# joeyee/Onet

Hardware: AMD Instinct MI355X
Metric: training images/sec (twin 256x256 pass) (higher is better)
Workload: dtype f32

## Files before the change

include/onet_hip.h:

```cpp
#ifndef ONET_HIP_H
#define ONET_HIP_H

#include <stdint.h>

#ifdef __cplusplus
extern "C" {
#endif

#define ONET_OK 0
#define ONET_EINVAL (-1)
#define ONET_EHIP (-2)

const char* onet_last_error(void);
int onet_abi_version(void);
int onet_device_info(int* cu_count, int* lds_bytes, int* wave_size, char* arch, int arch_len);

int onet_conv3x3_pack_weights(const float* w, float* wp_fwd, float* wp_dgrad,
                              int Cout, int Cin, void* stream);
int onet_convT2x2_pack_weights(const float* w, float* wp_fwd, float* wp_dgrad,
                               int Cin, int Cout, void* stream);
int onet_convT2x2_pack_weights_fused(const float* w, float* wq, int Cin, int Cout, void* stream);
int onet_convT2x2_fwd(const float* x, int64_t x_bs, const float* wq, const float* bias, float* y, int64_t y_bs,
                      int B, int Cin, int Ct, int h, int w, int Ho, int Wo, int pt, int pl, int operand_bf16,
        void* stream);
// ... 3 lines not shown
int64_t onet_convT2x2_dgrad_dbias_ws_bytes(int B, int Ct, int h, int w);
int onet_convT2x2_dgrad_dbias(const float* dy, int64_t dy_bs, const float* wp_dgrad, float* dx, int64_t dx_bs, float* dbias,
                              void* ws, int64_t ws_bytes, int B, int Cin, int Ct, int h, int w, int Ho, int Wo, int pt, int pl, int operand_bf16,
        void* stream);
int64_t onet_convT2x2_wgrad_ws_bytes(int B, int Cin, int Ct, int h, int w);
int onet_convT2x2_wgrad(const float* x, int64_t x_bs, const float* dy, int64_t dy_bs, float* dw, void* ws,
                        int64_t ws_bytes, int B, int Cin, int Ct, int h, int w, int Ho, int Wo, int pt, int pl, int operand_bf16,
        void* stream);
int onet_convT2x2_dbias(const float* dy, int64_t dy_bs, float* dbias, double* scratch, int accumulate, int B,
                        int C, int h, int w, int Ho, int Wo, int pt, int pl, void* stream);

int onet_conv_fwd(const float* x, int64_t x_bs, const float* wp, float* z, int64_t z_bs,
                  float* bn_part, int B, int Cin, int Cout, int H, int W, int ks, void* stream);
int onet_conv_fwd_nparts(int B, int Cout, int H, int W);

int onet_conv3x3_pack_weights_winograd4(const float* w, float* wq_fwd, float* wq_dgrad,
                                        int Cout, int Cin, void* stream);
int onet_conv3x3_winograd4_fwd(const float* x, int64_t x_bs, const float* wq, float* z, int64_t z_bs,
                               int B, int Cin, int Cout, int H, int W, void* stream);
int onet_conv3x3_winograd4_nparts(int B, int H, int W);
int onet_conv3x3_winograd4_fwd_stats(const float* x, int64_t x_bs, const float* wq, float* z, int64_t z_bs,
                                     float* part, int B, int Cin, int Cout, int H, int W, void* stream);
int onet_conv3x3_winograd4_dgrad_bnreduce(const float* dz, int64_t dz_bs, const float* wq_dgrad, float* da,
                                          int64_t da_bs, const float* z_prev, int64_t z_prev_bs,
                                          const float* save_prev, int group_images, float* part2,
                                          int B, int Cdz, int Cda, int H, int W, void* stream);
int onet_convT2x2_fwd_p(const float* x, int64_t x_bs, const float* wq, const float* bias, void* yP, int64_t yP_bs, const void* y_amax,
                        int nparts, int B, int Cin, int Ct, int h, int w, int Ho, int Wo, int pt, int pl, int operand_bf16, void* stream);
int onet_convT2x2_pack_weights_slots(const float* w, void* wP, void* wdP, void* amax_ws, int Cin, int Ct, int nparts, void* stream);
int onet_convT2x2_fwd_slots(const void* xP, int64_t xP_bs, const void* x_amax, const void* wP, const float* bias, void* yP, int64_t yP_bs,
                            const void* y_amax, int nparts, int B, int Cin, int Ct, int h, int w, void* stream);
int onet_convT2x2_dgrad_slots(const void* dyP, int64_t dyP_bs, const void* dy_amax, const void* wdP, float* dx, int64_t dx_bs, int nparts, int B,
                              int Cin, int Ct, int h, int w, void* stream);
int64_t onet_convT2x2_wgrad_slots_ws_bytes(int B, int Cin, int Ct, int h, int w);
int onet_convT2x2_wgrad_slots(const void* xP, int64_t xP_bs, const void* x_amax, const void* dyP, int64_t dyP_bs, const void* dy_amax, float* dw,
                              float* dbias, void* ws, int64_t ws_bytes, int nparts, int B, int Cin, int Ct, int h, int w, void* stream);
int onet_convT2x2_out_bound(const float* w, const float* bias, int Cin, int Ct, const void* x_amax, void* y_amax, void* stream);

int onet_conv3x3_split_pack_weights(const float* w, void* wq_fwd, void* wq_dgrad, void* amax_ws, int Cout, int Cin, int fwd_f16,
                                    int dgrad_f16, void* stream);
int onet_absmax_slots(const float* x, int64_t n, void* slots, void* stream);
int onet_conv3x3_split_conv_amax(const float* x, int64_t x_bs, const void* x_amax, int scale_always, const void* wq, float* z, int64_t z_bs,
                                 float* part, int B, int Cin, int Cout, int H, int W, void* stream);
int onet_conv3x3_split_wgrad_f16(const float* x, int64_t x_bs, const void* x_amax, const float* save, int n_groups, const float* dz,
                                 int64_t dz_bs, const void* dz_amax, float* dw, void* ws, int64_t ws_bytes, int B, int Cin, int Cout,
                                 int H, int W, int accumulate, void* stream);
int onet_conv3x3_split_fwd(const float* x, int64_t x_bs, const void* wq, int wq_f16, float* z, int64_t z_bs, int B, int Cin, int Cout,
                           int H, int W, void* stream);
int onet_conv3x3_split_nparts(int B, int H, int W);
int onet_split_pack_act(const float* x, int64_t x_bs, void* xs, int64_t xs_bs, int B, int C, int H, int W, int f16, float scale,
                        const void* slots ,
                        void* stream);
int onet_conv3x3_split_dgrad_pre_bnreduce(const void* dzs, int64_t dzs_bs, const void* dz_amax, int scale_always, const void* wq, int wq_f16,
                                          float* da, int64_t da_bs, const void* z_prev, int z_bf16, int64_t z_bs, const float* save, int group_images,
                                          float* rec4, void* da_amax, int B, int Cin, int Cout, int H, int W, void* stream);
int onet_conv3x3_split_fwd_pre(const void* xs, int64_t xs_bs, const void* x_amax, int scale_always, const void* x_amax2, int split_ch,
                               const void* wq, int wq_f16, void* z, int z_bf16 , int64_t z_bs,
                               float* part, int B, int Cin, int Cout, int H, int W,
                               void* stream);
int onet_conv3x3_split_dgrad_pre_slots(const void* dzs, int64_t dzs_bs, const void* dz_amax, int scale_always, const void* wq, int wq_f16,
                                       float* da, int64_t da_bs, void* daP, int64_t daP_bs, int ch0, const void* daP_amax, int B, int Cin,
                                       int Cout, int H, int W, void* stream);
int onet_conv3x3_dgrad_bound(const float* w, int Cout, int Cin, int ci0, const void* dz_amax, void* out_slots, void* stream);
int onet_conv3x3_split_fwd_pre_act(const void* xs, int64_t xs_bs, const void* x_amax, int scale_always, const void* x_amax2, int split_ch,
                                   const void* wq, const float* save, void* aP, int64_t aP_bs, const void* aP_slots, void* a_amax, float* a,
                                   int64_t a_bs, int B, int Cin, int Cout, int H, int W, void* stream);
// ... 145 lines not shown
```

onet_amd/csrc/convt_gemm.hip:

```cpp
#include <algorithm>
#include <cstdlib>
#include "common.hpp"

using namespace onet;

typedef float f32x16 __attribute__((ext_vector_type(16)));
typedef float f32x4g __attribute__((ext_vector_type(4)));
typedef float f32x2g __attribute__((ext_vector_type(2)));
typedef int i32x4g __attribute__((ext_vector_type(4)));
typedef __bf16 bf16x8g __attribute__((ext_vector_type(8)));
typedef __bf16 bf16x2g __attribute__((ext_vector_type(2)));
typedef unsigned u32x4g __attribute__((ext_vector_type(4)));

namespace {

__device__ __forceinline__ i32x4g g_rsrc(const void* base, int64_t bytes) {
    const uint64_t p = reinterpret_cast<uint64_t>(base);
    i32x4g r;
    r.x = (int)(p & 0xffffffffu);
    r.y = (int)((p >> 32) & 0xffffu);
    r.z = bytes > 0x7fffffffll ? 0x7fffffff : (int)bytes;
    r.w = 0x00020000;
    return r;
}
__device__ __forceinline__ unsigned g_lds(const float* p) {
    return (unsigned)(uintptr_t)(__attribute__((address_space(3))) const float*)p;
}
__device__ __forceinline__ void g_dma16(i32x4g rsrc, unsigned lds_base, unsigned voff) {
    unsigned keep;
    asm volatile("s_nop 4\n\ts_mov_b32 %0, m0\n\ts_mov_b32 m0, %3\n\ts_nop 0\n\tbuffer_load_dwordx4 %1, %2, 0 offen lds\n\ts_mov_b32 m0, %0"
                 : "=&s"(keep)
                 : "v"(voff), "s"(rsrc), "s"(lds_base)
                 : "memory");
// ... 424 lines not shown

__global__ __launch_bounds__(256) void convt_dbias_reduce_kernel(const float* __restrict__ part, float* __restrict__ db, int ntiles, int Ct) {
    const int c = blockIdx.x;
    double s = 0.0;
    for (int t = threadIdx.x; t < ntiles; t += 256) s += (double)part[(int64_t)t * Ct + c];
    __shared__ double sh[4];
    double v[1] = {s};
    block_sum_256<double, 1>(v, sh);
    if (threadIdx.x == 0) db[c] = (float)v[0];
}


typedef _Float16 f16x8g __attribute__((ext_vector_type(8)));

struct SArgs {
    const void* wP;
    const void* xP;
    int64_t x_bs;
    const float* bias;
    void* yP;
    int64_t y_bs;
    const unsigned* x_slots;
    const unsigned* y_slots;
    int B, Cin, Ct, h, w, mTiles, nTiles;
};

template <int NP>
__device__ __forceinline__ f32x16 s_mfma(u32x4g a, u32x4g b, f32x16 c) {
    if constexpr (NP == 2) return __builtin_amdgcn_mfma_f32_32x32x16_f16(__builtin_bit_cast(f16x8g, a), __builtin_bit_cast(f16x8g, b), c, 0, 0, 0);
    else return __builtin_amdgcn_mfma_f32_32x32x16_bf16(__builtin_bit_cast(bf16x8g, a), __builtin_bit_cast(bf16x8g, b), c, 0, 0, 0);
}

constexpr int SLOT_NST = 2, SLOT_OCC = 4;
template <int N>
__device__ __forceinline__ void slot_wait() {
    asm volatile("s_waitcnt vmcnt(%0)" ::"n"(N) : "memory");
}

template <int NP>
__global__ __launch_bounds__(256, SLOT_OCC) void convt_slot_fwd_kernel(SArgs g) {
    constexpr int KS = 4 / NP;
    constexpr int TILE = KS * NP * 128;
    constexpr int NPC = TILE / 256;
    constexpr int NST = SLOT_NST;
    __shared__ __attribute__((aligned(16))) u32x4g lds[NST * 2 * TILE];
    const int bid = xcd_block_id();
    const int mt = bid % g.mTiles;
    const int nt = bid / g.mTiles;
    const int tid = threadIdx.x, lane = tid & 63, wid = __builtin_amdgcn_readfirstlane(tid >> 6);
    const int wr = wid >> 1, wc = wid & 1, l31 = lane & 31, kh = lane >> 5;
    const int hw = g.h * g.w, M = 4 * g.Ct;
    const int m0 = mt * 128, n0 = nt * 128;
    const int b = n0 / hw, p0 = n0 % hw;

    const i32x4g ra = g_rsrc(g.wP, (int64_t)(g.Cin / 8) * NP * M * 16);
    const i32x4g rb = g_rsrc(reinterpret_cast<const unsigned*>(g.xP) + (int64_t)b * g.x_bs, (int64_t)(g.Cin / 8) * hw * NP * 16);
    unsigned a_off[NPC], b_off[NPC];
#pragma unroll
    for (int j = 0; j < NPC; ++j) {
        const int s = (wid * NPC + j) * 64 + lane;
        const int c8 = s / (NP * 128), part = (s >> 7) % NP, r = s & 127;
        a_off[j] = (unsigned)((((int64_t)c8 * NP + part) * M + m0 + r) * 16);
        const int p = p0 + r, i = p / g.w, jx = p % g.w;
        b_off[j] = (unsigned)(((((int64_t)c8 * g.h + i) * NP + part) * g.w + jx) * 16);
    }
    const unsigned a_step = (unsigned)((int64_t)KS * NP * M * 16), b_step = (unsigned)((int64_t)KS * hw * NP * 16);
    const unsigned lds0 = (unsigned)(uintptr_t)(__attribute__((address_space(3))) u32x4g*)lds;
    auto issue = [&](int chunk, int buf) __attribute__((always_inline)) {
        const unsigned la = lds0 + (unsigned)(buf * 2 * TILE * 16), lb = la + TILE * 16;
#pragma unroll
        for (int j = 0; j < NPC; ++j) g_dma16(ra, la + (wid * NPC + j) * 1024, a_off[j] + chunk * a_step);
#pragma unroll
        for (int j = 0; j < NPC; ++j) g_dma16(rb, lb + (wid * NPC + j) * 1024, b_off[j] + chunk * b_step);
    };
    static_assert(NST >= 2 && NST <= 4, "the tail waits below cover rings of two to four stages");

    f32x16 acc[2][2];
#pragma unroll
    for (int t = 0; t < 2; ++t)
#pragma unroll
        for (int u = 0; u < 2; ++u)
#pragma unroll
            for (int r = 0; r < 16; ++r) acc[t][u][r] = 0.f;

    const int nch = g.Cin / (8 * KS);
#pragma unroll
    for (int c = 0; c < NST - 1; ++c) issue(c, c);
    float undo = 1.f;
    if constexpr (NP == 2) {
        const float* meta = reinterpret_cast<const float*>(reinterpret_cast<const _Float16*>(g.wP) + (int64_t)NP * g.Cin * M);
        float x_inv;
        (void)amax_scale(amax_read(g.x_slots), false, x_inv);
        undo = meta[1] * x_inv;
    }
    float s_inv;
    const float s_up = NP == 1 ? 1.f : amax_scale(amax_read(g.y_slots), false, s_inv);
    float bsv[2][4];
#pragma unroll
    for (int t = 0; t < 2; ++t)
#pragma unroll
        for (int gq = 0; gq < 4; ++gq) bsv[t][gq] = g.bias ? g.bias[(m0 + wr * 64 + t * 32 + 8 * gq + 4 * kh) >> 2] : 0.f;
    slot_wait<(NST - 2) * 2 * NPC>();
    __syncthreads();
    for (int c = 0; c < nch; ++c) {
        const int buf = c % NST;
        if (c + NST - 1 < nch) issue(c + NST - 1, (c + NST - 1) % NST);
        const u32x4g* A = lds + buf * 2 * TILE + wr * 64 + l31;
        const u32x4g* Bt = lds + buf * 2 * TILE + TILE + wc * 64 + l31;
#pragma unroll
        for (int s = 0; s < KS / 2; ++s) {
            u32x4g af[2][NP], bf[2][NP];
#pragma unroll
            for (int t = 0; t < 2; ++t)
#pragma unroll
                for (int q = 0; q < NP; ++q) af[t][q] = A[((2 * s + kh) * NP + q) * 128 + t * 32];
#pragma unroll
            for (int u = 0; u < 2; ++u)
#pragma unroll
                for (int q = 0; q < NP; ++q) bf[u][q] = Bt[((2 * s + kh) * NP + q) * 128 + u * 32];
            if constexpr (NP == 2) {
#pragma unroll
                for (int t = 0; t < 2; ++t)
#pragma unroll
                    for (int u = 0; u < 2; ++u) acc[t][u] = s_mfma<NP>(af[t][1], bf[u][0], acc[t][u]);
#pragma unroll
                for (int t = 0; t < 2; ++t)
#pragma unroll
                    for (int u = 0; u < 2; ++u) acc[t][u] = s_mfma<NP>(af[t][0], bf[u][1], acc[t][u]);
            }
#pragma unroll
            for (int t = 0; t < 2; ++t)
#pragma unroll
                for (int u = 0; u < 2; ++u) acc[t][u] = s_mfma<NP>(af[t][0], bf[u][0], acc[t][u]);
        }
        const int behind = min(NST - 2, nch - 2 - c);
        constexpr int PPC = 2 * NPC;
        if (behind >= 2) slot_wait<2 * PPC>();
        else if (behind == 1) slot_wait<1 * PPC>();
        else slot_wait<0>();
        __syncthreads();
    }

#pragma unroll
    for (int t = 0; t < 2; ++t)
#pragma unroll
        for (int u = 0; u < 2; ++u) {
            const int p = p0 + wc * 64 + u * 32 + l31, y = p / g.w, x = p % g.w;
            const int c8 = (m0 + wr * 64 + t * 32) >> 5;
            float px[2][8];
#pragma unroll
            for (int gq = 0; gq < 4; ++gq) {
                const float bs = bsv[t][gq];
#pragma unroll
                for (int dj = 0; dj < 2; ++dj) {
                    const unsigned d0 = __builtin_bit_cast(unsigned, fmaf(acc[t][u][4 * gq + dj], undo, bs));
                    const unsigned d1 = __builtin_bit_cast(unsigned, fmaf(acc[t][u][4 * gq + 2 + dj], undo, bs));
                    const auto sw = __builtin_amdgcn_permlane32_swap(d0, d1, false, false);
                    const unsigned even = sw[0], odd = sw[1];
                    px[dj][2 * gq] = __builtin_bit_cast(float, even);
                    px[dj][2 * gq + 1] = __builtin_bit_cast(float, odd);
                }
            }
            u32x4g* dst = reinterpret_cast<u32x4g*>(reinterpret_cast<unsigned*>(g.yP) + (int64_t)b * g.y_bs) +
                          ((int64_t)(c8 * (2 * g.h) + 2 * y + kh) * NP) * (2 * g.w) + 2 * x;
#pragma unroll
            for (int dj = 0; dj < 2; ++dj) {
                u32x4g hi, mid;
#pragma unroll
                for (int k = 0; k < 4; ++k) {
                    if constexpr (NP == 2) {
                        unsigned hh, mm;
                        split2h_s(px[dj][2 * k], px[dj][2 * k + 1], s_up, hh, mm);
                        hi[k] = hh;
                        mid[k] = mm;
                    } else {
                        hi[k] = g_pack(px[dj][2 * k], px[dj][2 * k + 1]);
                    }
                }
                dst[dj] = hi;
                if constexpr (NP == 2) dst[2 * g.w + dj] = mid;
            }
        }
}

struct SDArgs {
    const void* wdP;
    const void* dyP;
    int64_t dy_bs;
    float* dx;
    int64_t dx_bs;
    const unsigned* dy_slots;
    int B, Cin, Ct, h, w, mTiles, nTiles;
};

template <int NP>
__global__ __launch_bounds__(256, SLOT_OCC) void convt_slot_dgrad_kernel(SDArgs g) {
    constexpr int KS = 4 / NP;
    constexpr int TILE = KS * NP * 128;
    constexpr int NPC = TILE / 256;
    constexpr int NST = SLOT_NST;
    __shared__ __attribute__((aligned(16))) u32x4g lds[NST * 2 * TILE];
    const int bid = xcd_block_id();
    const int mt = bid % g.mTiles, nt = bid / g.mTiles;
    const int tid = threadIdx.x, lane = tid & 63, wid = __builtin_amdgcn_readfirstlane(tid >> 6);
    const int wr = wid >> 1, wc = wid & 1, l31 = lane & 31, kh = lane >> 5;
    const int hw = g.h * g.w, M = g.Cin, Ho = 2 * g.h, Wo = 2 * g.w;
    const int m0 = mt * 128, n0 = nt * 128;
    const int b = n0 / hw, p0 = n0 % hw;

    const i32x4g ra = g_rsrc(g.wdP, (int64_t)(g.Ct / 2) * NP * M * 16);
    const i32x4g rb = g_rsrc(reinterpret_cast<const unsigned*>(g.dyP) + (int64_t)b * g.dy_bs, (int64_t)(g.Ct / 8) * Ho * NP * Wo * 16);
    unsigned a_off[NPC], b_px[NPC];
    int b_ks[NPC];
#pragma unroll
    for (int j = 0; j < NPC; ++j) {
        const int s = (wid * NPC + j) * 64 + lane;
        const int ks = s / (NP * 128), part = (s >> 7) % NP, r = s & 127;
        a_off[j] = (unsigned)((((int64_t)ks * NP + part) * M + m0 + r) * 16);
        const int p = p0 + r, i = p / g.w, jx = p % g.w;
        b_px[j] = (unsigned)(((((int64_t)2 * i) * NP + part) * Wo + 2 * jx) * 16);
        b_ks[j] = ks;
    }
    const unsigned a_step = (unsigned)((int64_t)KS * NP * M * 16);
    const unsigned lds0 = (unsigned)(uintptr_t)(__attribute__((address_space(3))) u32x4g*)lds;
    auto issue = [&](int chunk, int buf) __attribute__((always_inline)) {
        const unsigned la = lds0 + (unsigned)(buf * 2 * TILE * 16), lb = la + TILE * 16;
#pragma unroll
        for (int j = 0; j < NPC; ++j) g_dma16(ra, la + (wid * NPC + j) * 1024, a_off[j] + chunk * a_step);
#pragma unroll
        for (int j = 0; j < NPC; ++j) {
            const int kq = chunk * KS + b_ks[j], c8 = kq >> 2, di = (kq >> 1) & 1, dj = kq & 1;
            g_dma16(rb, lb + (wid * NPC + j) * 1024, b_px[j] + (unsigned)((((int64_t)c8 * Ho + di) * NP * Wo + dj) * 16));
        }
    };

    f32x16 acc[2][2];
#pragma unroll
    for (int t = 0; t < 2; ++t)
#pragma unroll
        for (int u = 0; u < 2; ++u)
#pragma unroll
            for (int r = 0; r < 16; ++r) acc[t][u][r] = 0.f;

    const int nch = (g.Ct / 2) / KS;
#pragma unroll
    for (int c = 0; c < NST - 1; ++c) issue(c, c);
    float undo = 1.f;
    if constexpr (NP == 2) {
        const float* meta = reinterpret_cast<const float*>(reinterpret_cast<const _Float16*>(g.wdP) + (int64_t)NP * 4 * g.Ct * M);
        float dy_inv;
        (void)amax_scale(amax_read(g.dy_slots), true, dy_inv);
        undo = meta[1] * dy_inv;
    }
    slot_wait<(NST - 2) * 2 * NPC>();
    __syncthreads();
    for (int c = 0; c < nch; ++c) {
        const int buf = c % NST;
        if (c + NST - 1 < nch) issue(c + NST - 1, (c + NST - 1) % NST);
        const u32x4g* A = lds + buf * 2 * TILE + wr * 64 + l31;
        const u32x4g* Bt = lds + buf * 2 * TILE + TILE + wc * 64 + l31;
#pragma unroll
        for (int s = 0; s < KS / 2; ++s) {
            u32x4g af[2][NP], bf[2][NP];
#pragma unroll
            for (int t = 0; t < 2; ++t)
#pragma unroll
                for (int q = 0; q < NP; ++q) af[t][q] = A[((2 * s + kh) * NP + q) * 128 + t * 32];
#pragma unroll
            for (int u = 0; u < 2; ++u)
#pragma unroll
                for (int q = 0; q < NP; ++q) bf[u][q] = Bt[((2 * s + kh) * NP + q) * 128 + u * 32];
            if constexpr (NP == 2) {
#pragma unroll
                for (int t = 0; t < 2; ++t)
#pragma unroll
                    for (int u = 0; u < 2; ++u) acc[t][u] = s_mfma<NP>(af[t][1], bf[u][0], acc[t][u]);
#pragma unroll
                for (int t = 0; t < 2; ++t)
#pragma unroll
                    for (int u = 0; u < 2; ++u) acc[t][u] = s_mfma<NP>(af[t][0], bf[u][1], acc[t][u]);
            }
#pragma unroll
            for (int t = 0; t < 2; ++t)
#pragma unroll
                for (int u = 0; u < 2; ++u) acc[t][u] = s_mfma<NP>(af[t][0], bf[u][0], acc[t][u]);
        }
        const int behind = min(NST - 2, nch - 2 - c);
        constexpr int PPC = 2 * NPC;
        if (behind >= 2) slot_wait<2 * PPC>();
        else if (behind == 1) slot_wait<1 * PPC>();
        else slot_wait<0>();
        __syncthreads();
    }
    float* xb = g.dx + (int64_t)b * g.dx_bs;
#pragma unroll
    for (int t = 0; t < 2; ++t)
#pragma unroll
        for (int u = 0; u < 2; ++u) {
            const int p = p0 + wc * 64 + u * 32 + l31;
#pragma unroll
            for (int r = 0; r < 16; ++r) {
                const int ci = m0 + wr * 64 + t * 32 + (r & 3) + 8 * (r >> 2) + 4 * kh;
                xb[(int64_t)ci * hw + p] = acc[t][u][r] * undo;
            }
        }
}

struct SWArgs {
    const void* xP;
    int64_t x_bs;
    const void* dyP;
    int64_t dy_bs;
    float* slab;
    float* db_part;
    const unsigned* x_slots;
    const unsigned* dy_slots;
    int B, Cin, Ct, h, w, lw;
    int mTiles, nTiles, splitK, chunksPerSplit;
};

constexpr int SW_CP = 32;
// ... 382 lines not shown
    if (rc) return rc;
    hipLaunchKernelGGL(convt_wgrad_reduce_kernel, dim3((unsigned)cdiv(n / 4, 256)), dim3(256), 0, st, (const float*)ws, dw, g.splitK,
                       n / 4, 0);
    return check_launch("convt_wgrad_reduce_kernel");
}

}

static bool wgrad_slots_plan(int B, int Cin, int Ct, int h, int w, int& splitK, int& per) {
    const bool big = (Cin % 256) == 0 && (Ct % 64) == 0;
    const int64_t chunks = (int64_t)B * h * w / SW_CP;
    const int64_t tiles = big ? (int64_t)(Cin / 256) * (Ct / 64) : (int64_t)(Cin / 128) * (Ct / 32);
    int64_t k = std::max<int64_t>(1, ((big ? 256 : 512) + tiles - 1) / tiles);
    k = std::min<int64_t>(k, std::max<int64_t>(1, chunks / (512 / SW_CP)));
    k = std::min<int64_t>(k, std::max<int64_t>(1, (256ll << 20) / ((int64_t)Cin * 4 * Ct * 4)));
    per = (int)((chunks + k - 1) / k);
    splitK = (int)((chunks + per - 1) / per);
    return big;
}

template <int NP, int BIG>
static int launch_wgrad_slots(SWArgs g, hipStream_t st) {
    using C = SwCfg<BIG>;
    const int lds = NP * (C::APL + C::BPL) * C::PXP * 16 * C::NST;
    auto kern = convt_slot_wgrad_kernel<NP, BIG>;
    static PerDeviceOnce once;
    if (once.first()) (void)hipFuncSetAttribute(reinterpret_cast<const void*>(kern), hipFuncAttributeMaxDynamicSharedMemorySize, lds);
    const int64_t blocks = (int64_t)g.splitK * g.mTiles * g.nTiles;
    ONET_REQUIRE(blocks > 0 && blocks < (1ll << 31), "convT2x2_wgrad_slots: grid too large");
    hipLaunchKernelGGL(kern, dim3((unsigned)blocks), dim3(C::NWAVE * 64), lds, st, g);
    return check_launch("convt_slot_wgrad_kernel");
}

extern "C" {

int onet_convT2x2_pack_weights_slots(const float* w, void* wP, void* wdP, void* amax_ws, int Cin, int Ct, int nparts, void* stream) {
    ONET_REQUIRE(w && wP && Cin > 0 && Ct > 0 && (Cin % 8) == 0 && (!wdP || (Ct % 8) == 0) && (nparts == 1 || nparts == 2),
                 "convT2x2_pack_weights_slots: bad args");
    ONET_REQUIRE(nparts == 1 || amax_ws, "convT2x2_pack_weights_slots: the fp16 pack needs the 8 KB magnitude workspace");
    hipStream_t st = as_stream(stream);
    const int64_t n = (int64_t)Cin * 4 * Ct;
    if (nparts == 2) {
        (void)hipMemsetAsync(amax_ws, 0, AMAX_SLOTS * AMAX_STRIDE * sizeof(unsigned), st);
        hipLaunchKernelGGL(convt_absmax_kernel, dim3((unsigned)std::min<int64_t>((n + 1023) / 1024, 1024)), dim3(256), 0, st, w, n, (unsigned*)amax_ws);
        int rc = check_launch("convt_absmax_kernel");
        if (rc) return rc;
    }
    hipLaunchKernelGGL(convt_pack_slots_kernel, dim3((unsigned)std::min<int64_t>(((wdP ? 2 : 1) * n + 255) / 256, 8192)), dim3(256), 0, st, w, wP,
                       wdP, Cin, Ct, nparts, (const unsigned*)amax_ws);
    return check_launch("convt_pack_slots_kernel");
}

int onet_convT2x2_dgrad_slots(const void* dyP, int64_t dyP_bs, const void* dy_amax, const void* wdP, float* dx, int64_t dx_bs, int nparts, int B,
                              int Cin, int Ct, int h, int w, void* stream) {
    ONET_REQUIRE(dyP && wdP && dx && B > 0 && Cin > 0 && Ct > 0 && h > 0 && w > 0 && (nparts == 1 || nparts == 2), "convT2x2_dgrad_slots: bad args");
    const int64_t hw = (int64_t)h * w;
    if ((Cin % 128) || (Ct % 32) || (hw % 128) || (w & 1) || !aligned16(dyP) || !aligned16(wdP) || (dyP_bs & 3) ||
        (int64_t)Ct * 4 * hw * 2 * nparts >= (1ll << 31) || (int64_t)Cin * 4 * Ct * 2 * nparts >= (1ll << 31))
        return 1;
    ONET_REQUIRE(dyP_bs >= (int64_t)Ct * 4 * hw * nparts / 2 && dx_bs >= (int64_t)Cin * hw, "convT2x2_dgrad_slots: batch stride too small");
    SDArgs g{wdP, dyP, dyP_bs, dx, dx_bs, (const unsigned*)dy_amax, B, Cin, Ct, h, w, Cin / 128, (int)(B * hw / 128)};
    const int64_t blocks = (int64_t)g.mTiles * g.nTiles;
    ONET_REQUIRE(blocks > 0 && blocks < (1ll << 31), "convT2x2_dgrad_slots: grid too large");
    if (nparts == 2) hipLaunchKernelGGL(convt_slot_dgrad_kernel<2>, dim3((unsigned)blocks), dim3(256), 0, as_stream(stream), g);
    else hipLaunchKernelGGL(convt_slot_dgrad_kernel<1>, dim3((unsigned)blocks), dim3(256), 0, as_stream(stream), g);
    return check_launch("convt_slot_dgrad_kernel");
}

int64_t onet_convT2x2_wgrad_slots_ws_bytes(int B, int Cin, int Ct, int h, int w) {
    if ((Cin % 128) || (Ct % 32) || (((int64_t)h * w) % 128) || (w & (w - 1))) return 0;
    int k, per;
    (void)wgrad_slots_plan(B, Cin, Ct, h, w, k, per);
    return (int64_t)k * ((int64_t)Cin * 4 * Ct + 4 * Ct) * 4;
}

int onet_convT2x2_wgrad_slots(const void* xP, int64_t xP_bs, const void* x_amax, const void* dyP, int64_t dyP_bs, const void* dy_amax, float* dw,
                              float* dbias, void* ws, int64_t ws_bytes, int nparts, int B, int Cin, int Ct, int h, int w, void* stream) {
    ONET_REQUIRE(xP && dyP && dw && ws && B > 0 && Cin > 0 && Ct > 0 && h > 0 && w > 0 && (nparts == 1 || nparts == 2), "convT2x2_wgrad_slots: bad args");
    const int64_t hw = (int64_t)h * w;
    if ((Cin % 128) || (Ct % 32) || (hw % 128) || (w & (w - 1)) || w < 2 || !aligned16(xP) || !aligned16(dyP) || !aligned16(dw) || (xP_bs & 3) ||
        (dyP_bs & 3) || (int64_t)Cin * hw * 2 * nparts >= (1ll << 31) || (int64_t)Ct * 4 * hw * 2 * nparts >= (1ll << 31))
        return 1;
    ONET_REQUIRE(xP_bs >= (int64_t)Cin * hw * nparts / 2 && dyP_bs >= (int64_t)Ct * 4 * hw * nparts / 2, "convT2x2_wgrad_slots: batch stride too small");
    int lw = 0;
    while ((1 << lw) < w) ++lw;
    SWArgs g{xP, xP_bs, dyP, dyP_bs, (float*)ws, nullptr, (const unsigned*)x_amax, (const unsigned*)dy_amax, B, Cin, Ct, h, w, lw, 0, 0, 1, 0};
    const bool big = wgrad_slots_plan(B, Cin, Ct, h, w, g.splitK, g.chunksPerSplit);
    g.mTiles = big ? Cin / 256 : Cin / 128;
    g.nTiles = big ? Ct / 64 : Ct / 32;
    const int64_t n = (int64_t)Cin * 4 * Ct;
    ONET_REQUIRE(ws_bytes >= (int64_t)g.splitK * (n + 4 * Ct) * 4, "convT2x2_wgrad_slots: workspace too small (onet_convT2x2_wgrad_slots_ws_bytes)");
    if (dbias) g.db_part = (float*)ws + (int64_t)g.splitK * n;
    hipStream_t st = as_stream(stream);
    int rc;
    if (nparts == 2) rc = big ? launch_wgrad_slots<2, 1>(g, st) : launch_wgrad_slots<2, 0>(g, st);
    else rc = big ? launch_wgrad_slots<1, 1>(g, st) : launch_wgrad_slots<1, 0>(g, st);
    if (rc) return rc;
    hipLaunchKernelGGL(convt_wgrad_reduce_kernel, dim3((unsigned)cdiv(n / 4, 256)), dim3(256), 0, st, (const float*)ws, dw, g.splitK, n / 4, 0);
    rc = check_launch("convt_wgrad_reduce_kernel");
    if (rc || !dbias) return rc;
    hipLaunchKernelGGL(convt_dbias_reduce_kernel, dim3((unsigned)Ct), dim3(256), 0, st, (const float*)g.db_part, dbias, g.splitK * 4, Ct);
    return check_launch("convt_dbias_reduce_kernel");
}

int onet_convT2x2_fwd_slots(const void* xP, int64_t xP_bs, const void* x_amax, const void* wP, const float* bias, void* yP, int64_t yP_bs,
                            const void* y_amax, int nparts, int B, int Cin, int Ct, int h, int w, void* stream) {
    ONET_REQUIRE(xP && wP && yP && B > 0 && Cin > 0 && Ct > 0 && h > 0 && w > 0 && (nparts == 1 || nparts == 2), "convT2x2_fwd_slots: bad args");
    const int64_t hw = (int64_t)h * w;
    if ((Cin % 32) || Cin < 128 || (Ct % 32) || (hw % 128) || (w & 1) || !aligned16(xP) || !aligned16(wP) || !aligned16(yP) || (xP_bs & 3) || (yP_bs & 3) ||
        (int64_t)Cin * hw * 2 * nparts >= (1ll << 31) || (int64_t)Cin * 4 * Ct * 2 * nparts >= (1ll << 31))
        return 1;
    ONET_REQUIRE(xP_bs >= (int64_t)Cin * hw * nparts / 2 && yP_bs >= (int64_t)Ct * 4 * hw * nparts / 2, "convT2x2_fwd_slots: batch stride too small");
    SArgs g{wP, xP, xP_bs, bias, yP, yP_bs, (const unsigned*)x_amax, (const unsigned*)y_amax, B, Cin, Ct, h, w, (4 * Ct) / 128, (int)(B * hw / 128)};
    const int64_t blocks = (int64_t)g.mTiles * g.nTiles;
    ONET_REQUIRE(blocks > 0 && blocks < (1ll << 31), "convT2x2_fwd_slots: grid too large");
    if (nparts == 2) hipLaunchKernelGGL(convt_slot_fwd_kernel<2>, dim3((unsigned)blocks), dim3(256), 0, as_stream(stream), g);
    else hipLaunchKernelGGL(convt_slot_fwd_kernel<1>, dim3((unsigned)blocks), dim3(256), 0, as_stream(stream), g);
    return check_launch("convt_slot_fwd_kernel");
}

}
```

onet_amd/ops.py:

```python
from __future__ import annotations

import torch

from . import _lib

F32 = torch.float32


import os as _os


def _flags_from_env():
    out = {}
    for item in _os.environ.get("ONET_FLAGS", "").split(","):
        if "=" in item:
            k, v = item.split("=", 1)
            out[k.strip()] = v.strip()
    return out


_FLAGS = _flags_from_env()


def _flag(name, default):
# ... 307 lines not shown

def convT2x2_fwd(x, wq, bias, out, Ct, pt, pl):
    require_gpu(x, wq, out)
    x, xbs = plane(x)
    B, Cin, h, w = x.shape
    Ho, Wo = out.shape[2], out.shape[3]
    obs = out.stride(0) if B > 1 else Ct * Ho * Wo
    e0 = _prof_begin("convt_gemm_kernel")
    _lib.call("onet_convT2x2_fwd", _p(x), xbs, _p(wq), _p(bias), _p(out), obs, B, Cin, Ct, h, w, Ho, Wo, pt, pl,
              convt_operand_bf16(B, h, w, Ct), _stream())
    _prof_end("convt_gemm_kernel", 2.0 * B * h * w * Cin * 4 * Ct, e0, 4.0 * (B * h * w * (Cin + 4 * Ct) + 4 * Cin * Ct))


def convT2x2_out_bound(weight, bias, x_amax):
    w = weight.detach()
    w = w if w.is_contiguous() else w.contiguous()
    slots = new_amax(w.device)
    _lib.call("onet_convT2x2_out_bound", _p(w), _p(bias), w.shape[0], w.shape[1], _p(x_amax), _p(slots), _stream())
    return slots


def packT2x2_slots(w, parts=2, dgrad=False):
    require_gpu(w)
    w = w.detach().contiguous()
    Cin, Ct = w.shape[0], w.shape[1]
    dt = torch.float16 if parts == 2 else BF
    wP = torch.empty(Cin * 4 * Ct * parts + 4, dtype=dt, device=w.device)
    wdP = torch.empty(Cin * 4 * Ct * parts + 4, dtype=dt, device=w.device) if dgrad else None
    ws = torch.empty(2048, dtype=torch.int32, device=w.device) if parts == 2 else None
    _lib.call("onet_convT2x2_pack_weights_slots", _p(w), _p(wP), _p(wdP), _p(ws), Cin, Ct, parts, _stream())
    return (wP, wdP) if dgrad else wP


def convT2x2_dgrad_slots(dyP, wdP, Cin, dy_slots=None):
    B, C8, Ho, parts, Wo, _ = dyP.shape
    Ct, h, w = C8 * 8, Ho // 2, Wo // 2
    dx = torch.empty((B, Cin, h, w), dtype=F32, device=dyP.device)
    e0 = _prof_begin("convt_gemm_kernel")
    rc = _lib.load().onet_convT2x2_dgrad_slots(_p(dyP), _pbs(dyP), _p(dy_slots), _p(wdP), _p(dx), Cin * h * w, parts, B, Cin, Ct, h, w, _stream())
    flops, nb = 2.0 * B * h * w * Cin * 4 * Ct, B * h * w * (4.0 * Cin + 2.0 * parts * 4 * Ct)
    _prof_end("convt_gemm_kernel", flops if rc == 0 else 0.0, e0, nb if rc == 0 else 0.0)
    if rc < 0:
        raise _lib.OnetHipError(f"onet_convT2x2_dgrad_slots failed ({rc}): {_lib.last_error()}")
    return dx if rc == 0 else None


def convT2x2_wgrad_slots(xP, dyP, dw_shape, x_slots=None, dy_slots=None, want_dbias=False, out=None, db_out=None):
    B, C8, h, parts, w, _ = xP.shape
    Cin, Ct = C8 * 8, dyP.shape[1] * 8
    assert tuple(dw_shape) == (Cin, Ct, 2, 2) and dyP.shape[3] == parts and dyP.shape[2] == 2 * h and xP.dtype == dyP.dtype
    need = int(_lib.load().onet_convT2x2_wgrad_slots_ws_bytes(B, Cin, Ct, h, w))
    if need <= 0:
        return None
    ws = workspace(need, xP.device)
    dw = out if out is not None else torch.empty(dw_shape, dtype=F32, device=xP.device)
    db = (db_out if db_out is not None else torch.empty(Ct, dtype=F32, device=xP.device)) if want_dbias else None
    e0 = _prof_begin("convt_wgrad_gemm_kernel")
    rc = _lib.load().onet_convT2x2_wgrad_slots(_p(xP), _pbs(xP), _p(x_slots), _p(dyP), _pbs(dyP), _p(dy_slots), _p(dw), _p(db), _p(ws),
                                               ws.numel() * 4, parts, B, Cin, Ct, h, w, _stream())
    flops, nb = 2.0 * B * h * w * Cin * 4 * Ct, 2.0 * parts * B * h * w * (Cin + 4 * Ct)
    _prof_end("convt_wgrad_gemm_kernel", flops if rc == 0 else 0.0, e0, nb if rc == 0 else 0.0)
    if rc < 0:
        raise _lib.OnetHipError(f"onet_convT2x2_wgrad_slots failed ({rc}): {_lib.last_error()}")
    return (dw, db) if rc == 0 else None


def conv3x3_dgrad_bound(weight, dz_slots, ci0):
    w = weight.detach()
    w = w if w.is_contiguous() else w.contiguous()
    slots = new_amax(w.device)
# ... 59 lines not shown
                               f"{self._v} instead")

    def __getitem__(self, i):
        if self._t[i] is None:
            self._same_weight()
            self._t[i] = packT2x2_fused(self.w) if i == 0 else packT2x2(self.w)[1]
        return self._t[i]

    def __iter__(self):
        return iter((_LazyPack(self, 0), _LazyPack(self, 1)))

    def __len__(self):
        return 2

    def slots(self, parts):
        if parts not in self._s:
            self._same_weight()
            self._s[parts] = packT2x2_slots(self.w, parts, dgrad=bool(CONVT_BWD_SLOTS))
        v = self._s[parts]
        return v[0] if isinstance(v, tuple) else v

    def dgrad_slots(self, parts):
        v = self._s.get(parts)
        if not isinstance(v, tuple):
            self._same_weight()
            self._s[parts] = v = packT2x2_slots(self.w, parts, dgrad=True)
        return v[1]


def convT2x2_fwd_slots(xP, wP, bias, outP, Ct, x_slots=None, slots=None, kind="convt_gemm_kernel"):
    B, C8, h, parts, w, _ = xP.shape
    assert outP.shape[3] == parts and outP.shape[2] == 2 * h and outP.shape[4] == 2 * w and xP.dtype == wP.dtype == outP.dtype
    Cin = C8 * 8
    e0 = _prof_begin(kind)
    rc = _lib.load().onet_convT2x2_fwd_slots(_p(xP), _pbs(xP), _p(x_slots), _p(wP), _p(bias), _p(outP), _pbs(outP), _p(slots), parts, B, Cin, Ct,
                                             h, w, _stream())
    eb = 2.0 * parts
    flops, nb = 2.0 * B * h * w * Cin * 4 * Ct, eb * (B * h * w * (Cin + 4 * Ct) + 4 * Cin * Ct)
    _prof_end(kind, flops if rc == 0 else 0.0, e0, nb if rc == 0 else 0.0)
    if rc < 0:
        raise _lib.OnetHipError(f"onet_convT2x2_fwd_slots failed ({rc}): {_lib.last_error()}")
    return rc == 0


def convT2x2_fwd_p(x, wq, bias, outP, Ct, pt, pl, slots=None):
    require_gpu(x, wq)
    x, xbs = plane(x)
    B, Cin, h, w = x.shape
    Ho, Wo = outP.shape[2], outP.shape[4]
    e0 = _prof_begin("convt_gemm_kernel")
    rc = _lib.load().onet_convT2x2_fwd_p(_p(x), xbs, _p(wq), _p(bias), _p(outP), _pbs(outP), _p(slots), outP.shape[3], B, Cin, Ct, h, w, Ho, Wo, pt, pl,
                                         convt_operand_bf16(B, h, w, Ct), _stream())
    flops, nb = 2.0 * B * h * w * Cin * 4 * Ct, 4.0 * (B * h * w * (Cin + 4 * Ct) + 4 * Cin * Ct)
    _prof_end("convt_gemm_kernel", flops if rc == 0 else 0.0, e0, nb if rc == 0 else 0.0)
    if rc < 0:
        raise _lib.OnetHipError(f"onet_convT2x2_fwd_p failed ({rc}): {_lib.last_error()}")
    return rc == 0


import os as _os
CONV_ALGO = _os.environ.get("ONET_CONV_ALGO", "auto")
TWIN = _flag("TWIN", True)


BF = torch.bfloat16

# ... 1322 lines not shown
```

Measured before the change: 602.2.

## Add wide 256x128 tile variant for convT slot fwd/dgrad kernels with LDS-staged stores

```diff
diff --git a/include/onet_hip.h b/include/onet_hip.h
--- a/include/onet_hip.h
+++ b/include/onet_hip.h
@@ -59,6 +59,7 @@
                             const void* y_amax, int nparts, int B, int Cin, int Ct, int h, int w, void* stream);
 int onet_convT2x2_dgrad_slots(const void* dyP, int64_t dyP_bs, const void* dy_amax, const void* wdP, float* dx, int64_t dx_bs, int nparts, int B,
                               int Cin, int Ct, int h, int w, void* stream);
+int onet_convT2x2_slots_wide_tile(int enable);
 int64_t onet_convT2x2_wgrad_slots_ws_bytes(int B, int Cin, int Ct, int h, int w);
 int onet_convT2x2_wgrad_slots(const void* xP, int64_t xP_bs, const void* x_amax, const void* dyP, int64_t dyP_bs, const void* dy_amax, float* dw,
                               float* dbias, void* ws, int64_t ws_bytes, int nparts, int B, int Cin, int Ct, int h, int w, void* stream);
diff --git a/onet_amd/csrc/convt_gemm.hip b/onet_amd/csrc/convt_gemm.hip
--- a/onet_amd/csrc/convt_gemm.hip
+++ b/onet_amd/csrc/convt_gemm.hip
@@ -1,4 +1,5 @@
 #include <algorithm>
+#include <atomic>
 #include <cstdlib>
 #include "common.hpp"
 
@@ -489,46 +490,66 @@
 }
 
 constexpr int SLOT_NST = 2, SLOT_OCC = 4;
+template <int WM> struct SlotTile {
+    static constexpr int NW = WM * 2, NT = 64 * NW;
+    static constexpr int BM = 64 * WM, BN = 128;
+    static constexpr int OCC = SLOT_OCC * 4 / NW;
+    static constexpr int NST = WM == 2 ? SLOT_NST : 3;
+    static constexpr int LDS = NST * 4 * (BM + BN) * 16;
+    static constexpr bool STG = WM == 4;
+};
 template <int N>
 __device__ __forceinline__ void slot_wait() {
     asm volatile("s_waitcnt vmcnt(%0)" ::"n"(N) : "memory");
 }
 
-template <int NP>
-__global__ __launch_bounds__(256, SLOT_OCC) void convt_slot_fwd_kernel(SArgs g) {
+template <int NP, int WM>
+__global__ __launch_bounds__((SlotTile<WM>::NT), (SlotTile<WM>::OCC)) void convt_slot_fwd_kernel(SArgs g) {
+    using T = SlotTile<WM>;
     constexpr int KS = 4 / NP;
-    constexpr int TILE = KS * NP * 128;
-    constexpr int NPC = TILE / 256;
-    constexpr int NST = SLOT_NST;
-    __shared__ __attribute__((aligned(16))) u32x4g lds[NST * 2 * TILE];
+    constexpr int BM = T::BM, BN = T::BN;
+    constexpr bool STG = T::STG;
+    constexpr int TILE_A = KS * NP * BM, TILE_B = KS * NP * BN;
+    constexpr int STAGE = TILE_A + TILE_B;
+    constexpr int NPA = TILE_A / 64 / T::NW, NPB = TILE_B / 64 / T::NW;
+    static_assert(NPA * 64 * T::NW == TILE_A && NPB * 64 * T::NW == TILE_B, "the waves share the DMA pieces evenly");
+    constexpr int NST = T::NST;
+    static_assert(NST * STAGE * 16 == T::LDS, "the launcher's LDS size");
+    extern __shared__ __attribute__((aligned(16))) unsigned char slot_smem[];
+    u32x4g* lds = reinterpret_cast<u32x4g*>(slot_smem);
     const int bid = xcd_block_id();
     const int mt = bid % g.mTiles;
     const int nt = bid / g.mTiles;
     const int tid = threadIdx.x, lane = tid & 63, wid = __builtin_amdgcn_readfirstlane(tid >> 6);
     const int wr = wid >> 1, wc = wid & 1, l31 = lane & 31, kh = lane >> 5;
     const int hw = g.h * g.w, M = 4 * g.Ct;
-    const int m0 = mt * 128, n0 = nt * 128;
+    const int m0 = mt * BM, n0 = nt * BN;
     const int b = n0 / hw, p0 = n0 % hw;
 
     const i32x4g ra = g_rsrc(g.wP, (int64_t)(g.Cin / 8) * NP * M * 16);
     const i32x4g rb = g_rsrc(reinterpret_cast<const unsigned*>(g.xP) + (int64_t)b * g.x_bs, (int64_t)(g.Cin / 8) * hw * NP * 16);
-    unsigned a_off[NPC], b_off[NPC];
-#pragma unroll
-    for (int j = 0; j < NPC; ++j) {
-        const int s = (wid * NPC + j) * 64 + lane;
-        const int c8 = s / (NP * 128), part = (s >> 7) % NP, r = s & 127;
+    unsigned a_off[NPA], b_off[NPB];
+#pragma unroll
+    for (int j = 0; j < NPA; ++j) {
+        const int s = (wid * NPA + j) * 64 + lane;
+        const int c8 = s / (NP * BM), part = (s / BM) % NP, r = s % BM;
         a_off[j] = (unsigned)((((int64_t)c8 * NP + part) * M + m0 + r) * 16);
+    }
+#pragma unroll
+    for (int j = 0; j < NPB; ++j) {
+        const int s = (wid * NPB + j) * 64 + lane;
+        const int c8 = s / (NP * BN), part = (s / BN) % NP, r = s % BN;
         const int p = p0 + r, i = p / g.w, jx = p % g.w;
         b_off[j] = (unsigned)(((((int64_t)c8 * g.h + i) * NP + part) * g.w + jx) * 16);
     }
     const unsigned a_step = (unsigned)((int64_t)KS * NP * M * 16), b_step = (unsigned)((int64_t)KS * hw * NP * 16);
-    const unsigned lds0 = (unsigned)(uintptr_t)(__attribute__((address_space(3))) u32x4g*)lds;
+    const unsigned lds0 = (unsigned)(uintptr_t)(__attribute__((address_space(3))) unsigned char*)slot_smem;
     auto issue = [&](int chunk, int buf) __attribute__((always_inline)) {
-        const unsigned la = lds0 + (unsigned)(buf * 2 * TILE * 16), lb = la + TILE * 16;
-#pragma unroll
-        for (int j = 0; j < NPC; ++j) g_dma16(ra, la + (wid * NPC + j) * 1024, a_off[j] + chunk * a_step);
-#pragma unroll
-        for (int j = 0; j < NPC; ++j) g_dma16(rb, lb + (wid * NPC + j) * 1024, b_off[j] + chunk * b_step);
+        const unsigned la = lds0 + (unsigned)(buf * STAGE * 16), lb = la + TILE_A * 16;
+#pragma unroll
+        for (int j = 0; j < NPA; ++j) g_dma16(ra, la + (wid * NPA + j) * 1024, a_off[j] + chunk * a_step);
+#pragma unroll
+        for (int j = 0; j < NPB; ++j) g_dma16(rb, lb + (wid * NPB + j) * 1024, b_off[j] + chunk * b_step);
     };
     static_assert(NST >= 2 && NST <= 4, "the tail waits below cover rings of two to four stages");
 
@@ -557,24 +578,24 @@
     for (int t = 0; t < 2; ++t)
 #pragma unroll
         for (int gq = 0; gq < 4; ++gq) bsv[t][gq] = g.bias ? g.bias[(m0 + wr * 64 + t * 32 + 8 * gq + 4 * kh) >> 2] : 0.f;
-    slot_wait<(NST - 2) * 2 * NPC>();
+    slot_wait<(NST - 2) * (NPA + NPB)>();
     __syncthreads();
     for (int c = 0; c < nch; ++c) {
         const int buf = c % NST;
         if (c + NST - 1 < nch) issue(c + NST - 1, (c + NST - 1) % NST);
-        const u32x4g* A = lds + buf * 2 * TILE + wr * 64 + l31;
-        const u32x4g* Bt = lds + buf * 2 * TILE + TILE + wc * 64 + l31;
+        const u32x4g* A = lds + buf * STAGE + wr * 64 + l31;
+        const u32x4g* Bt = lds + buf * STAGE + TILE_A + wc * 64 + l31;
 #pragma unroll
         for (int s = 0; s < KS / 2; ++s) {
             u32x4g af[2][NP], bf[2][NP];
 #pragma unroll
             for (int t = 0; t < 2; ++t)
 #pragma unroll
-                for (int q = 0; q < NP; ++q) af[t][q] = A[((2 * s + kh) * NP + q) * 128 + t * 32];
+                for (int q = 0; q < NP; ++q) af[t][q] = A[((2 * s + kh) * NP + q) * BM + t * 32];
 #pragma unroll
             for (int u = 0; u < 2; ++u)
 #pragma unroll
-                for (int q = 0; q < NP; ++q) bf[u][q] = Bt[((2 * s + kh) * NP + q) * 128 + u * 32];
+                for (int q = 0; q < NP; ++q) bf[u][q] = Bt[((2 * s + kh) * NP + q) * BN + u * 32];
             if constexpr (NP == 2) {
 #pragma unroll
                 for (int t = 0; t < 2; ++t)
@@ -591,7 +612,7 @@
                 for (int u = 0; u < 2; ++u) acc[t][u] = s_mfma<NP>(af[t][0], bf[u][0], acc[t][u]);
         }
         const int behind = min(NST - 2, nch - 2 - c);
-        constexpr int PPC = 2 * NPC;
+        constexpr int PPC = NPA + NPB;
         if (behind >= 2) slot_wait<2 * PPC>();
         else if (behind == 1) slot_wait<1 * PPC>();
         else slot_wait<0>();
@@ -618,8 +639,9 @@
                     px[dj][2 * gq + 1] = __builtin_bit_cast(float, odd);
                 }
             }
-            u32x4g* dst = reinterpret_cast<u32x4g*>(reinterpret_cast<unsigned*>(g.yP) + (int64_t)b * g.y_bs) +
-                          ((int64_t)(c8 * (2 * g.h) + 2 * y + kh) * NP) * (2 * g.w) + 2 * x;
+            u32x4g* yb = reinterpret_cast<u32x4g*>(reinterpret_cast<unsigned*>(g.yP) + (int64_t)b * g.y_bs);
+            u32x4g* dst = yb + ((int64_t)(c8 * (2 * g.h) + 2 * y + kh) * NP) * (2 * g.w) + 2 * x;
+            u32x4g* stg = lds + wid * (NP * 128);
 #pragma unroll
             for (int dj = 0; dj < 2; ++dj) {
                 u32x4g hi, mid;
@@ -634,8 +656,27 @@
                         hi[k] = g_pack(px[dj][2 * k], px[dj][2 * k + 1]);
                     }
                 }
-                dst[dj] = hi;
-                if constexpr (NP == 2) dst[2 * g.w + dj] = mid;
+                if constexpr (STG) {
+                    stg[kh * 64 + 2 * l31 + dj] = hi;
+                    if constexpr (NP == 2) stg[128 + kh * 64 + 2 * l31 + dj] = mid;
+                } else {
+                    dst[dj] = hi;
+                    if constexpr (NP == 2) dst[2 * g.w + dj] = mid;
+                }
+            }
+            if constexpr (STG) {
+                __builtin_amdgcn_fence(__ATOMIC_RELEASE, "wavefront");
+                __builtin_amdgcn_wave_barrier();
+                __builtin_amdgcn_fence(__ATOMIC_ACQUIRE, "wavefront");
+                const int ps = p0 + wc * 64 + u * 32 + (lane >> 1), ys = ps / g.w, xs = ps % g.w;
+                u32x4g* ds = yb + ((int64_t)(c8 * (2 * g.h) + 2 * ys) * NP) * (2 * g.w) + 2 * xs + (lane & 1);
+#pragma unroll
+                for (int di = 0; di < 2; ++di)
+#pragma unroll
+                    for (int q = 0; q < NP; ++q) ds[(di * NP + q) * (2 * g.w)] = stg[q * 128 + di * 64 + lane];
+                __builtin_amdgcn_fence(__ATOMIC_RELEASE, "wavefront");
+                __builtin_amdgcn_wave_barrier();
+                __builtin_amdgcn_fence(__ATOMIC_ACQUIRE, "wavefront");
             }
         }
 }
@@ -650,44 +691,54 @@
     int B, Cin, Ct, h, w, mTiles, nTiles;
 };
 
-template <int NP>
-__global__ __launch_bounds__(256, SLOT_OCC) void convt_slot_dgrad_kernel(SDArgs g) {
+template <int NP, int WM>
+__global__ __launch_bounds__((SlotTile<WM>::NT), (SlotTile<WM>::OCC)) void convt_slot_dgrad_kernel(SDArgs g) {
+    using T = SlotTile<WM>;
     constexpr int KS = 4 / NP;
-    constexpr int TILE = KS * NP * 128;
-    constexpr int NPC = TILE / 256;
-    constexpr int NST = SLOT_NST;
-    __shared__ __attribute__((aligned(16))) u32x4g lds[NST * 2 * TILE];
+    constexpr int BM = T::BM, BN = T::BN;
+    constexpr int TILE_A = KS * NP * BM, TILE_B = KS * NP * BN, STAGE = TILE_A + TILE_B;
+    constexpr int NPA = TILE_A / 64 / T::NW, NPB = TILE_B / 64 / T::NW;
+    static_assert(NPA * 64 * T::NW == TILE_A && NPB * 64 * T::NW == TILE_B, "the waves share the DMA pieces evenly");
+    constexpr int NST = T::NST;
+    static_assert(NST * STAGE * 16 == T::LDS, "the launcher's LDS size");
+    extern __shared__ __attribute__((aligned(16))) unsigned char slot_smem[];
+    u32x4g* lds = reinterpret_cast<u32x4g*>(slot_smem);
     const int bid = xcd_block_id();
     const int mt = bid % g.mTiles, nt = bid / g.mTiles;
     const int tid = threadIdx.x, lane = tid & 63, wid = __builtin_amdgcn_readfirstlane(tid >> 6);
     const int wr = wid >> 1, wc = wid & 1, l31 = lane & 31, kh = lane >> 5;
     const int hw = g.h * g.w, M = g.Cin, Ho = 2 * g.h, Wo = 2 * g.w;
-    const int m0 = mt * 128, n0 = nt * 128;
+    const int m0 = mt * BM, n0 = nt * BN;
     const int b = n0 / hw, p0 = n0 % hw;
 
     const i32x4g ra = g_rsrc(g.wdP, (int64_t)(g.Ct / 2) * NP * M * 16);
     const i32x4g rb = g_rsrc(reinterpret_cast<const unsigned*>(g.dyP) + (int64_t)b * g.dy_bs, (int64_t)(g.Ct / 8) * Ho * NP * Wo * 16);
-    unsigned a_off[NPC], b_px[NPC];
-    int b_ks[NPC];
-#pragma unroll
-    for (int j = 0; j < NPC; ++j) {
-        const int s = (wid * NPC + j) * 64 + lane;
-        const int ks = s / (NP * 128), part = (s >> 7) % NP, r = s & 127;
+    unsigned a_off[NPA], b_px[NPB];
+    int b_ks[NPB];
+#pragma unroll
+    for (int j = 0; j < NPA; ++j) {
+        const int s = (wid * NPA + j) * 64 + lane;
+        const int ks = s / (NP * BM), part = (s / BM) % NP, r = s % BM;
         a_off[j] = (unsigned)((((int64_t)ks * NP + part) * M + m0 + r) * 16);
+    }
+#pragma unroll
+    for (int j = 0; j < NPB; ++j) {
+        const int s = (wid * NPB + j) * 64 + lane;
+        const int ks = s / (NP * BN), part = (s / BN) % NP, r = s % BN;
         const int p = p0 + r, i = p / g.w, jx = p % g.w;
         b_px[j] = (unsigned)(((((int64_t)2 * i) * NP + part) * Wo + 2 * jx) * 16);
         b_ks[j] = ks;
     }
     const unsigned a_step = (unsigned)((int64_t)KS * NP * M * 16);
-    const unsigned lds0 = (unsigned)(uintptr_t)(__attribute__((address_space(3))) u32x4g*)lds;
+    const unsigned lds0 = (unsigned)(uintptr_t)(__attribute__((address_space(3))) unsigned char*)slot_smem;
     auto issue = [&](int chunk, int buf) __attribute__((always_inline)) {
-        const unsigned la = lds0 + (unsigned)(buf * 2 * TILE * 16), lb = la + TILE * 16;
-#pragma unroll
-        for (int j = 0; j < NPC; ++j) g_dma16(ra, la + (wid * NPC + j) * 1024, a_off[j] + chunk * a_step);
-#pragma unroll
-        for (int j = 0; j < NPC; ++j) {
+        const unsigned la = lds0 + (unsigned)(buf * STAGE * 16), lb = la + TILE_A * 16;
+#pragma unroll
+        for (int j = 0; j < NPA; ++j) g_dma16(ra, la + (wid * NPA + j) * 1024, a_off[j] + chunk * a_step);
+#pragma unroll
+        for (int j = 0; j < NPB; ++j) {
             const int kq = chunk * KS + b_ks[j], c8 = kq >> 2, di = (kq >> 1) & 1, dj = kq & 1;
-            g_dma16(rb, lb + (wid * NPC + j) * 1024, b_px[j] + (unsigned)((((int64_t)c8 * Ho + di) * NP * Wo + dj) * 16));
+            g_dma16(rb, lb + (wid * NPB + j) * 1024, b_px[j] + (unsigned)((((int64_t)c8 * Ho + di) * NP * Wo + dj) * 16));
         }
     };
 
@@ -709,24 +760,24 @@
         (void)amax_scale(amax_read(g.dy_slots), true, dy_inv);
         undo = meta[1] * dy_inv;
     }
-    slot_wait<(NST - 2) * 2 * NPC>();
+    slot_wait<(NST - 2) * (NPA + NPB)>();
     __syncthreads();
     for (int c = 0; c < nch; ++c) {
         const int buf = c % NST;
         if (c + NST - 1 < nch) issue(c + NST - 1, (c + NST - 1) % NST);
-        const u32x4g* A = lds + buf * 2 * TILE + wr * 64 + l31;
-        const u32x4g* Bt = lds + buf * 2 * TILE + TILE + wc * 64 + l31;
+        const u32x4g* A = lds + buf * STAGE + wr * 64 + l31;
+        const u32x4g* Bt = lds + buf * STAGE + TILE_A + wc * 64 + l31;
 #pragma unroll
         for (int s = 0; s < KS / 2; ++s) {
             u32x4g af[2][NP], bf[2][NP];
 #pragma unroll
             for (int t = 0; t < 2; ++t)
 #pragma unroll
-                for (int q = 0; q < NP; ++q) af[t][q] = A[((2 * s + kh) * NP + q) * 128 + t * 32];
+                for (int q = 0; q < NP; ++q) af[t][q] = A[((2 * s + kh) * NP + q) * BM + t * 32];
 #pragma unroll
             for (int u = 0; u < 2; ++u)
 #pragma unroll
-                for (int q = 0; q < NP; ++q) bf[u][q] = Bt[((2 * s + kh) * NP + q) * 128 + u * 32];
+                for (int q = 0; q < NP; ++q) bf[u][q] = Bt[((2 * s + kh) * NP + q) * BN + u * 32];
             if constexpr (NP == 2) {
 #pragma unroll
                 for (int t = 0; t < 2; ++t)
@@ -743,7 +794,7 @@
                 for (int u = 0; u < 2; ++u) acc[t][u] = s_mfma<NP>(af[t][0], bf[u][0], acc[t][u]);
         }
         const int behind = min(NST - 2, nch - 2 - c);
-        constexpr int PPC = 2 * NPC;
+        constexpr int PPC = NPA + NPB;
         if (behind >= 2) slot_wait<2 * PPC>();
         else if (behind == 1) slot_wait<1 * PPC>();
         else slot_wait<0>();
@@ -1192,7 +1243,50 @@
     return check_launch("convt_slot_wgrad_kernel");
 }
 
+static std::atomic<int> g_slot_wide{1};
+
+template <int WM>
+static int launch_slot_fwd(SArgs g, int nparts, hipStream_t st) {
+    using T = SlotTile<WM>;
+    g.mTiles = 4 * g.Ct / T::BM;
+    g.nTiles = (int)((int64_t)g.B * g.h * g.w / T::BN);
+    const int64_t blocks = (int64_t)g.mTiles * g.nTiles;
+    ONET_REQUIRE(blocks > 0 && blocks < (1ll << 31), "convT2x2_fwd_slots: grid too large");
+    auto k2 = convt_slot_fwd_kernel<2, WM>;
+    auto k1 = convt_slot_fwd_kernel<1, WM>;
+    static PerDeviceOnce once;
+    if (T::LDS > 65536 && once.first()) {
+        (void)hipFuncSetAttribute(reinterpret_cast<const void*>(k2), hipFuncAttributeMaxDynamicSharedMemorySize, T::LDS);
+        (void)hipFuncSetAttribute(reinterpret_cast<const void*>(k1), hipFuncAttributeMaxDynamicSharedMemorySize, T::LDS);
+    }
+    hipLaunchKernelGGL(nparts == 2 ? k2 : k1, dim3((unsigned)blocks), dim3(T::NT), T::LDS, st, g);
+    return check_launch("convt_slot_fwd_kernel");
+}
+
+template <int WM>
+static int launch_slot_dgrad(SDArgs g, int nparts, hipStream_t st) {
+    using T = SlotTile<WM>;
+    g.mTiles = g.Cin / T::BM;
+    g.nTiles = (int)((int64_t)g.B * g.h * g.w / T::BN);
+    const int64_t blocks = (int64_t)g.mTiles * g.nTiles;
+    ONET_REQUIRE(blocks > 0 && blocks < (1ll << 31), "convT2x2_dgrad_slots: grid too large");
+    auto k2 = convt_slot_dgrad_kernel<2, WM>;
+    auto k1 = convt_slot_dgrad_kernel<1, WM>;
+    static PerDeviceOnce once;
+    if (T::LDS > 65536 && once.first()) {
+        (void)hipFuncSetAttribute(reinterpret_cast<const void*>(k2), hipFuncAttributeMaxDynamicSharedMemorySize, T::LDS);
+        (void)hipFuncSetAttribute(reinterpret_cast<const void*>(k1), hipFuncAttributeMaxDynamicSharedMemorySize, T::LDS);
+    }
+    hipLaunchKernelGGL(nparts == 2 ? k2 : k1, dim3((unsigned)blocks), dim3(T::NT), T::LDS, st, g);
+    return check_launch("convt_slot_dgrad_kernel");
+}
+
 extern "C" {
+
+int onet_convT2x2_slots_wide_tile(int enable) {
+    g_slot_wide.store(enable, std::memory_order_relaxed);
+    return 0;
+}
 
 int onet_convT2x2_pack_weights_slots(const float* w, void* wP, void* wdP, void* amax_ws, int Cin, int Ct, int nparts, void* stream) {
     ONET_REQUIRE(w && wP && Cin > 0 && Ct > 0 && (Cin % 8) == 0 && (!wdP || (Ct % 8) == 0) && (nparts == 1 || nparts == 2),
@@ -1219,12 +1313,9 @@
         (int64_t)Ct * 4 * hw * 2 * nparts >= (1ll << 31) || (int64_t)Cin * 4 * Ct * 2 * nparts >= (1ll << 31))
         return 1;
     ONET_REQUIRE(dyP_bs >= (int64_t)Ct * 4 * hw * nparts / 2 && dx_bs >= (int64_t)Cin * hw, "convT2x2_dgrad_slots: batch stride too small");
-    SDArgs g{wdP, dyP, dyP_bs, dx, dx_bs, (const unsigned*)dy_amax, B, Cin, Ct, h, w, Cin / 128, (int)(B * hw / 128)};
-    const int64_t blocks = (int64_t)g.mTiles * g.nTiles;
-    ONET_REQUIRE(blocks > 0 && blocks < (1ll << 31), "convT2x2_dgrad_slots: grid too large");
-    if (nparts == 2) hipLaunchKernelGGL(convt_slot_dgrad_kernel<2>, dim3((unsigned)blocks), dim3(256), 0, as_stream(stream), g);
-    else hipLaunchKernelGGL(convt_slot_dgrad_kernel<1>, dim3((unsigned)blocks), dim3(256), 0, as_stream(stream), g);
-    return check_launch("convt_slot_dgrad_kernel");
+    SDArgs g{wdP, dyP, dyP_bs, dx, dx_bs, (const unsigned*)dy_amax, B, Cin, Ct, h, w, 0, 0};
+    const bool wide = g_slot_wide.load(std::memory_order_relaxed) != 0 && (Cin % 256) == 0;
+    return wide ? launch_slot_dgrad<4>(g, nparts, as_stream(stream)) : launch_slot_dgrad<2>(g, nparts, as_stream(stream));
 }
 
 int64_t onet_convT2x2_wgrad_slots_ws_bytes(int B, int Cin, int Ct, int h, int w) {
@@ -1271,12 +1362,9 @@
         (int64_t)Cin * hw * 2 * nparts >= (1ll << 31) || (int64_t)Cin * 4 * Ct * 2 * nparts >= (1ll << 31))
         return 1;
     ONET_REQUIRE(xP_bs >= (int64_t)Cin * hw * nparts / 2 && yP_bs >= (int64_t)Ct * 4 * hw * nparts / 2, "convT2x2_fwd_slots: batch stride too small");
-    SArgs g{wP, xP, xP_bs, bias, yP, yP_bs, (const unsigned*)x_amax, (const unsigned*)y_amax, B, Cin, Ct, h, w, (4 * Ct) / 128, (int)(B * hw / 128)};
-    const int64_t blocks = (int64_t)g.mTiles * g.nTiles;
-    ONET_REQUIRE(blocks > 0 && blocks < (1ll << 31), "convT2x2_fwd_slots: grid too large");
-    if (nparts == 2) hipLaunchKernelGGL(convt_slot_fwd_kernel<2>, dim3((unsigned)blocks), dim3(256), 0, as_stream(stream), g);
-    else hipLaunchKernelGGL(convt_slot_fwd_kernel<1>, dim3((unsigned)blocks), dim3(256), 0, as_stream(stream), g);
-    return check_launch("convt_slot_fwd_kernel");
-}
-
-}
+    SArgs g{wP, xP, xP_bs, bias, yP, yP_bs, (const unsigned*)x_amax, (const unsigned*)y_amax, B, Cin, Ct, h, w, 0, 0};
+    const bool wide = g_slot_wide.load(std::memory_order_relaxed) != 0 && ((4 * Ct) % 256) == 0;
+    return wide ? launch_slot_fwd<4>(g, nparts, as_stream(stream)) : launch_slot_fwd<2>(g, nparts, as_stream(stream));
+}
+
+}
diff --git a/onet_amd/ops.py b/onet_amd/ops.py
--- a/onet_amd/ops.py
+++ b/onet_amd/ops.py
@@ -363,10 +363,23 @@
     return (wP, wdP) if dgrad else wP
 
 
+CONVT_WIDE = _flag("CONVT_WIDE", True)
+_convt_wide_sent = None
+
+
+def _convt_wide_sync():
+    global _convt_wide_sent
+    v = int(CONVT_WIDE)
+    if v != _convt_wide_sent:
+        _lib.load().onet_convT2x2_slots_wide_tile(v)
+        _convt_wide_sent = v
+
+
 def convT2x2_dgrad_slots(dyP, wdP, Cin, dy_slots=None):
     B, C8, Ho, parts, Wo, _ = dyP.shape
     Ct, h, w = C8 * 8, Ho // 2, Wo // 2
     dx = torch.empty((B, Cin, h, w), dtype=F32, device=dyP.device)
+    _convt_wide_sync()
     e0 = _prof_begin("convt_gemm_kernel")
     rc = _lib.load().onet_convT2x2_dgrad_slots(_p(dyP), _pbs(dyP), _p(dy_slots), _p(wdP), _p(dx), Cin * h * w, parts, B, Cin, Ct, h, w, _stream())
     flops, nb = 2.0 * B * h * w * Cin * 4 * Ct, B * h * w * (4.0 * Cin + 2.0 * parts * 4 * Ct)
@@ -492,6 +505,7 @@
     B, C8, h, parts, w, _ = xP.shape
     assert outP.shape[3] == parts and outP.shape[2] == 2 * h and outP.shape[4] == 2 * w and xP.dtype == wP.dtype == outP.dtype
     Cin = C8 * 8
+    _convt_wide_sync()
     e0 = _prof_begin(kind)
     rc = _lib.load().onet_convT2x2_fwd_slots(_p(xP), _pbs(xP), _p(x_slots), _p(wP), _p(bias), _p(outP), _pbs(outP), _p(slots), parts, B, Cin, Ct,
                                              h, w, _stream())
```

Result: no change. 601.7 (-0.1%).
